# rongzhao-zhang/EfficientQ

Measured on AMD Instinct MI355X. Metric: ptq_calibration_throughput, higher is better.
Workload: dtype i8xi8->i32 (exact) for the Gram systems and per-iteration loss convs of the layers with quantised input, f32/f64 elsewhere

## Files before the change

efficientq_amd/_lib.py:

```python
from __future__ import annotations

import ctypes as C
import os

import torch

_HERE = os.path.dirname(os.path.abspath(__file__))
LIB_PATH = os.path.join(_HERE, "libeffq_hip.so")

EFFQ_OK = 0
_ERR_NAMES = {1: "EFFQ_ERR_ARG", 2: "EFFQ_ERR_HIP", 3: "EFFQ_ERR_WORKSPACE", 4: "EFFQ_ERR_NO_DEVICE",
              5: "EFFQ_ERR_NOT_CONVERGED"}


class EffqError(RuntimeError):
    pass


class Geom(C.Structure):
    _fields_ = [(n, C.c_int32) for n in
                ("N", "C1", "C2", "D", "H", "W", "KD", "KH", "KW", "SD", "SH", "SW", "PD", "PH", "PW")]

    def out_dims(self):
        return ((self.D + 2 * self.PD - self.KD) // self.SD + 1,
# ... 72 lines not shown
    "effq_fp_bracket_update": (_I, [_SZ, _I, _D, _D, _D, _I, _P, _P, _P]),
    "effq_fp_traj_max": (_SZ, []),
    "effq_fp_traj_ws_bytes": (_SZ, [_SZ]),
    "effq_spd_inverse_prepare": (_I, [_P]),
    "effq_fp_traj_pred_bytes": (_SZ, []),
    "effq_fixed_point_traj": (_I, [_P, _P, _P, _SZ, _I, _D, _D, _D, _I, _P, _P, _P, _SZ, _P]),
    "effq_fixed_point_bucket_rec": (_I, [_P, _P, _P, _SZ, _I, _D, _D, _D, _I, _P, _P, _SZ, _P, _P]),
    "effq_fixed_point_coop_rec": (_I, [_P, _P, _P, _SZ, _I, _D, _D, _D, _I, _P, _P, _P, _P]),
    "effq_fp_check": (_I, [_P, _P, _P]),
    "effq_fp_channels_max_row": (_I, []),
    "effq_fixed_point_channels": (_I, [_P, _P, _P, _I, _I, _I, _D, _I, _P, _P, _P, _P]),
    "effq_fixed_point_channels_proj": (_I, [_P, _P, _P, _I, _I, _I, _D, _I, _P, _P, _P, _P, _F, _P, _P, _P, _I, _I, _D,
                                            _D, _P]),
    "effq_gram_packed_elems": (_SZ, [_I, _I]),
    "effq_gram_pack": (_I, [_P, _P, _I, _I, _P, _P]),
    "effq_gram_unpack": (_I, [_P, _I, _I, _P, _P, _P]),
    "effq_act_quant_backward": (_I, [_P, _P, _I, _P, _P, _P, _SZ, _P, _P]),
    "effq_att_classes_ws_bytes": (_SZ, []),
    "effq_att_classes": (_I, [_P, _LL, _P, _P, _P, C.POINTER(C.c_int32), _P, _P]),
    "effq_prof_enable": (_I, [_I]),
    "effq_prof_count": (_I, []),
    "effq_prof_read": (_I, [_I, C.POINTER(ProfRecord)]),
    "effq_admm_num_inverses": (_I, [_D, _D, _I, _I]),
    "effq_admm_run": (_I, [C.POINTER(AdmmRunArgs)]),
    "effq_admm_select_best": (_I, [_P, _I, _P, _P, _SZ, _SZ, _P, _P, _P, _P]),
    "effq_gram_ws_bytes": (_SZ, [_GP, _I]),
    "effq_gram_accum": (_I, [_P, _P, _P, _GP, _I, _P, _P, _I, _P, _SZ, _P]),
    "effq_gram_plan_query": (_I, [_GP, _I, _IP, _IP, _IP, _IP, _LLP, _IP, _IP]),
    "effq_gram_i8_supported": (_I, [_GP, _I]),
    "effq_gram_i8_ws_bytes": (_SZ, [_GP, _I]),
    "effq_gram_accum_i8": (_I, [_P, _P, _GP, _I, _P, _I, _P, _P, _P, _I, _LL, _P, _P, _I, _P, _SZ, _P]),
    "effq_gram_accum_i8_unw": (_I, [_P, _P, _GP, _I, _P, _I, _P, _P, _P, _I, _LL, _P, _P, _I, _P, _P, _P, _SZ, _P]),
    "effq_gram_i8_plan_query": (_I, [_GP, _I, _LL, _IP, _IP, _IP, _IP, _IP, _IP]),
    "effq_upsample_trilinear": (_I, [_P, _I, _I, _I, _I, _I, _I, _I, _I, _P, _P]),
    "effq_gram_f64_supported": (_I, [_GP, _I]),
    "effq_gram_f64_ws_bytes": (_SZ, [_GP, _I]),
    "effq_gram_f64": (_I, [_P, _P, _GP, _I, _P, _P, _P, _SZ, _P]),
    "effq_gram_f64_plan_query": (_I, [_GP, _I, _IP, _IP, _IP, _IP]),
    "effq_gram_loss_ws_bytes": (_SZ, [_I]),
    "effq_gram_loss": (_I, [_P, _P, _P, _P, _P, _I, _I, _I, _P, _P, _SZ, _P]),
    "effq_packed_bytes": (_SZ, [_SZ, _I]),
    "effq_pack_levels": (_I, [_P, _SZ, _I, _P, _P]),
    "effq_unpack_levels": (_I, [_P, _SZ, _I, _P, _P]),
    "effq_ainv_ld": (_I, [_I]),
    "effq_fp_bracket_export_words": (_SZ, []),
    "effq_fp_bracket_export": (_I, [_P, _SZ, _P, _P, _SZ, _P]),
    "effq_fp_bracket_rebase": (_I, [_P, _P, _SZ, _P]),
    "effq_fp_bracket_import": (_I, [_P, _SZ, _P, _I, _SZ, _P, _P, _SZ, _P]),
    "effq_admm_uses_traj": (_I, [_SZ, _I]),
    "effq_gram_loss_i8_supported": (_I, [_I, _I, _I, _I]),
    "effq_gram_loss_i8_num_planes": (_I, [C.c_longlong]),
    "effq_gram_loss_i8_planes_bytes": (_SZ, [_I, _I, _I]),
    "effq_gram_loss_i8_prepare": (_I, [_P, _I, _I, _P, _I, _I, _P, _P, _P]),
    "effq_gram_loss_i8_ws_bytes": (_SZ, []),
    "effq_gram_loss_i8": (_I, [_P, _I, _P, _P, _P, _P, _P, _P, _P, _I, _I, _I, _I, _I, _I, _P, _P, _SZ, _P]),
    "effq_spd_inverse_ws_bytes": (_SZ, [_I]),
    "effq_spd_inverse": (_I, [_P, _I, _I, _D, _D, _P, _P, _SZ, _P]),
    "effq_spd_inverse_plan": (_I, [_I, _IP, _IP, _IP]),
    "effq_prox_plan_query": (_I, [_I, _I, _IP, _IP, _IP, _IP]),
    "effq_prox_ws_bytes": (_SZ, [_I, _I]),
    "effq_prox_solve": (_I, [_P, _P, _P, _P, _P, _P, _I, _I, _I, _D, _D, _P, _P, _P, _SZ, _P]),
    "effq_prox_solve_shifted": (_I, [_P, _P, _P, _P, _P, _P, _I, _I, _I, _D, _D, _D, _I, _P, _P, _P, _SZ, _P]),
    "effq_admm_presum": (_I, [_P, _P, _P, _SZ, _P]),
    "effq_admm_project_dual": (_I, [_P, _P, _P, _I, _P, _P, _F, _P, _SZ, _P]),
    "effq_conv_i8_supported": (_I, [_GP, _I, _I]),
    "effq_conv_i8s_supported": (_I, [_GP, _I, _I]),
# ... 84 lines not shown
```

efficientq_amd/csrc/gram_i8.hip:

```cpp
#include <stdint.h>
#include <stdlib.h>
#include "common.h"

namespace effq {

typedef int gi_v4i __attribute__((ext_vector_type(4)));
typedef int gi_v16i __attribute__((ext_vector_type(16)));

constexpr int GI_KC = 128;
constexpr int GI_MB = 128;
constexpr int GI_RS = GI_KC + 16;
constexpr int GI_T = 256;
constexpr int GI_PANEL = GI_MB * GI_RS;
constexpr int GI_LDS = 4 * GI_PANEL + 2 * GI_KC * 16;
constexpr int GI_MAXCLS = 16;
constexpr int GI_MAX_CPS = 1000;

struct GramI8Params {
  const uint8_t* x;
  const int8_t* yd;
  const int* vox_list;
  const int* chunk_cls;
  const int* vtab;
  int N, C1, C2, C2P, D, H, W, OD, OH, OW;
  int KD, KH, KW, SD, SH, SW, PD, PH, PW;
  int T, RX, YR0, E, NB, NBX, npairs;
  long long V;
  int nchunks, nsplit, cps, ncls;
  long long* slabs;
  int debug;
};

__device__ __forceinline__ void gi_transpose4(int r0, int r1, int r2, int r3, int (&o)[4]) {
  const int t0 = __builtin_amdgcn_perm(r1, r0, 0x05010400);
  const int t1 = __builtin_amdgcn_perm(r1, r0, 0x07030602);
  const int t2 = __builtin_amdgcn_perm(r3, r2, 0x05010400);
  const int t3 = __builtin_amdgcn_perm(r3, r2, 0x07030602);
  o[0] = __builtin_amdgcn_perm(t2, t0, 0x05040100);
  o[1] = __builtin_amdgcn_perm(t2, t0, 0x07060302);
  o[2] = __builtin_amdgcn_perm(t3, t1, 0x05040100);
  o[3] = __builtin_amdgcn_perm(t3, t1, 0x07060302);
}

__device__ __forceinline__ gi_v4i gi_build_entry(const GramI8Params& p, int v) {
  gi_v4i e = {0, 0, 0, 0};
  if (v < 0) return e;
  int t = v;
  const int ow = t % p.OW;
  t /= p.OW;
  const int oh = t % p.OH;
  t /= p.OH;
  const int od = t % p.OD;
  const int n = t / p.OD;
  const int id0 = od * p.SD - p.PD, ih0 = oh * p.SH - p.PH, iw0 = ow * p.SW - p.PW;
  unsigned m = 0x80000000u;
  int tap = 0;
  for (int kd = 0; kd < p.KD; ++kd)
    for (int kh = 0; kh < p.KH; ++kh)
      for (int kw = 0; kw < p.KW; ++kw, ++tap) {
        const int id = id0 + kd, ih = ih0 + kh, iw = iw0 + kw;
        const bool ok = id >= 0 && id < p.D && ih >= 0 && ih < p.H && iw >= 0 && iw < p.W;
        m |= (ok ? 1u : 0u) << tap;
      }
  e[0] = ((n * p.D + id0) * p.H + ih0) * p.W + iw0;
  e[1] = (int)m;
  e[2] = v;
  return e;
}

__global__ __launch_bounds__(256) void k_gi_voxtable(GramI8Params p, gi_v4i* __restrict__ table) {
  const long long nslots = (long long)p.nchunks * GI_KC;
  const long long stride = (long long)gridDim.x * blockDim.x;
  for (long long s = (long long)blockIdx.x * blockDim.x + threadIdx.x; s < nslots; s += stride) {
    const int v = (p.vox_list != nullptr) ? p.vox_list[s] : ((s < p.V) ? (int)s : -1);
    table[s] = gi_build_entry(p, v);
  }
}

__global__ __launch_bounds__(GI_T, 2) void k_gram_i8(GramI8Params p) {
  extern __shared__ __attribute__((aligned(16))) unsigned char gi_smem[];
  unsigned char* const panI = gi_smem;
  unsigned char* const panJ = gi_smem + 2 * GI_PANEL;
  gi_v4i* const tbl = reinterpret_cast<gi_v4i*>(gi_smem + 4 * GI_PANEL);

  const int tid = threadIdx.x, lane = tid & 63, wid = tid >> 6;
  const int li = lane & 31, lh = lane >> 5;
  const int wr = wid >> 1, wc = wid & 1;

  int I = 0, rem = blockIdx.x;
  while (rem >= p.NB - I) {
    rem -= p.NB - I;
    ++I;
  }
  const int J = I + rem;
  const bool diag = (I == J);

  const int c_begin = blockIdx.y * p.cps;
  const int c_end = min(c_begin + p.cps, p.nchunks);
  if (c_begin >= c_end) return;

  const int vg = tid & 31, rg = tid >> 5;
  int kindI, tapI, offI, kindJ, tapJ, offJ;
  auto make_rg = [&](int r0, int& kind, int& tap, int& off) {
    kind = 3;
    tap = 0;
    off = 0;
    if (r0 < p.RX) {
      kind = 0;
      tap = r0 / p.C1;
      const int c0 = r0 - tap * p.C1;
      const int kw = tap % p.KW, t2 = tap / p.KW;
      const int kh = t2 % p.KH, kd = t2 / p.KH;
      off = ((kd * p.H + kh) * p.W + kw) * p.C1 + c0;
    } else if (r0 == p.RX) {
      kind = 2;
    } else if (r0 >= p.YR0 && r0 < p.E) {
      kind = 1;
      off = r0 - p.YR0;
    }
  };
  make_rg(I * GI_MB + 16 * rg, kindI, tapI, offI);
  make_rg(J * GI_MB + 16 * rg, kindJ, tapJ, offJ);
  const unsigned char* const srcI = (kindI == 1) ? reinterpret_cast<const unsigned char*>(p.yd) : p.x;
  const unsigned char* const srcJ = (kindJ == 1) ? reinterpret_cast<const unsigned char*>(p.yd) : p.x;
  const int ystride = 4 * p.C2P;

  const gi_v4i* const vtab = reinterpret_cast<const gi_v4i*>(p.vtab);

  gi_v4i vI[4], vJ[4];
  unsigned okI = 0, okJ = 0;
#define GI_FETCH(val, okb, kind, tap, off, src, slot)                                            \
  {                                                                                              \
    okb = 0;                                                                                     \
    _Pragma("unroll") for (int q = 0; q < 4; ++q) {                                              \
      const gi_v4i e = tbl[(slot) * GI_KC + vg + 32 * q];                                        \
      const unsigned m = (unsigned)e[1];                                                         \
      const unsigned okx = (m >> (tap)) & 1u, okv = m >> 31;                                     \
      const unsigned ok = (kind == 0) ? okx : ((kind <= 2) ? okv : 0u);                          \
      const int ax = okx ? (e[0] * p.C1 + (off)) : 0;                                            \
      const int ay = e[2] * ystride + (off);                                                     \
      const int addr = (kind == 0) ? ax : ((kind == 1) ? ay : 0);                                \
      val[q] = *reinterpret_cast<const gi_v4i*>(src + ((EFFQ_DBG(p) == 2) ? 0 : addr));             \
      okb |= ok << q;                                                                            \
    }                                                                                            \
  }
  auto stage = [&](unsigned char* P, gi_v4i (&val)[4], unsigned okb, int kind) {
#pragma unroll
    for (int q = 0; q < 4; ++q) {
      const bool ok = (okb >> q) & 1u;
      gi_v4i z = {0, 0, 0, 0};
      if (kind == 2) z[0] = 1;
      if (!ok || kind >= 2) val[q] = ok ? z : gi_v4i{0, 0, 0, 0};
    }
#pragma unroll
    for (int k = 0; k < 4; ++k) {
      int o[4];
      gi_transpose4(val[0][k], val[1][k], val[2][k], val[3][k], o);
#pragma unroll
      for (int b = 0; b < 4; ++b) *reinterpret_cast<int*>(P + (16 * rg + 4 * k + b) * GI_RS + 4 * vg) = o[b];
    }
  };

  gi_v16i acc[2][2];
#pragma unroll
  for (int m = 0; m < 2; ++m)
#pragma unroll
    for (int n = 0; n < 2; ++n)
#pragma unroll
      for (int r = 0; r < 16; ++r) acc[m][n][r] = 0;
  const bool live = (I * GI_MB + wr * 64 < p.E) && (J * GI_MB + wc * 64 < p.E);

  auto flush = [&](int cls) {
    long long* S = p.slabs + ((size_t)cls * p.npairs + blockIdx.x) * (size_t)(GI_MB * GI_MB);
#pragma unroll
    for (int m = 0; m < 2; ++m)
#pragma unroll
      for (int n = 0; n < 2; ++n)
#pragma unroll
        for (int r = 0; r < 16; ++r) {
          const int row = wr * 64 + m * 32 + (r & 3) + 8 * (r >> 2) + 4 * lh;
          const int col = wc * 64 + n * 32 + li;
          const int v = acc[m][n][r];
          if (v != 0)
            atomicAdd(reinterpret_cast<unsigned long long*>(&S[row * GI_MB + col]), (unsigned long long)(long long)v);
          acc[m][n][r] = 0;
        }
  };

  {
    const int k = tid & (GI_KC - 1);
    const int cc = (tid < GI_KC) ? c_begin : min(c_begin + 1, c_end - 1);
    tbl[(tid < GI_KC ? 0 : 1) * GI_KC + k] = vtab[(size_t)cc * GI_KC + k];
  }
  __syncthreads();
// ... 11 lines not shown
    const int b = (c - c_begin) & 1;
    const int c2 = min(c + 2, c_end - 1);
    const int cls_raw = clsp[has_cls ? c2 : 0];
    const gi_v4i traw = vtab[(size_t)c2 * GI_KC + (tid & (GI_KC - 1))];
    GI_FETCH(vI, okI, kindI, tapI, offI, srcI, b ^ 1)
    if (!diag) GI_FETCH(vJ, okJ, kindJ, tapJ, offJ, srcJ, b ^ 1)
    __builtin_amdgcn_sched_barrier(0);
    if (live && EFFQ_DBG(p) != 1) {
      const unsigned char* PI = panI + b * GI_PANEL + (wr * 64 + li) * GI_RS + lh * 16;
      const unsigned char* PJ = (diag ? panI : panJ) + b * GI_PANEL + (wc * 64 + li) * GI_RS + lh * 16;
#pragma unroll
      for (int s = 0; s < GI_KC / 32; ++s) {
        gi_v4i a[2], bb[2];
#pragma unroll
        for (int m = 0; m < 2; ++m) a[m] = *reinterpret_cast<const gi_v4i*>(PI + m * 32 * GI_RS + s * 32);
#pragma unroll
        for (int n = 0; n < 2; ++n) bb[n] = *reinterpret_cast<const gi_v4i*>(PJ + n * 32 * GI_RS + s * 32);
#pragma unroll
        for (int m = 0; m < 2; ++m)
#pragma unroll
          for (int n = 0; n < 2; ++n) acc[m][n] = __builtin_amdgcn_mfma_i32_32x32x32_i8(a[m], bb[n], acc[m][n], 0, 0, 0);
      }
    }
    if (cls_next != cls_cur && live) flush(cls_cur);
    if (tid < GI_KC) tbl[b * GI_KC + tid] = traw;
    if (EFFQ_DBG(p) != 3) {
      stage(panI + (b ^ 1) * GI_PANEL, vI, okI, kindI);
      if (!diag) stage(panJ + (b ^ 1) * GI_PANEL, vJ, okJ, kindJ);
    }
    cls_cur = cls_next;
    cls_next = (c + 2 < c_end) ? (has_cls ? cls_raw : 0) : -1;
    __syncthreads();
  }
#undef GI_FETCH
}

__global__ __launch_bounds__(256) void k_gi_absmax(const float* __restrict__ y, size_t n, unsigned* __restrict__ out) {
  float m = 0.0f;
  const size_t stride = (size_t)gridDim.x * blockDim.x;
  for (size_t e = (size_t)blockIdx.x * blockDim.x + threadIdx.x; e < n; e += stride) m = fmaxf(m, fabsf(y[e]));
#pragma unroll
  for (int o = 32; o > 0; o >>= 1) m = fmaxf(m, __shfl_xor(m, o));
  if ((threadIdx.x & 63) == 0) atomicMax(out, __float_as_uint(m));
}

__device__ __forceinline__ int gi_y_exponent(unsigned ymax_bits) {
  const float ymax = __uint_as_float(ymax_bits);
  int ex = 0;
  if (ymax > 0.0f && ymax < 3.0e38f) (void)frexpf(ymax, &ex);
  return ex < -90 ? -90 : ex;
}

__global__ __launch_bounds__(256) void k_gi_ydigits(const float* __restrict__ y, long long V, int C2, int C2P,
                                                    const unsigned* __restrict__ ymax_bits, int8_t* __restrict__ yd) {
  const int ex = gi_y_exponent(*ymax_bits);
  const float scale = ldexpf(1.0f, 30 - ex);
  const size_t tot = (size_t)V * C2P, stride = (size_t)gridDim.x * blockDim.x;
  for (size_t e = (size_t)blockIdx.x * blockDim.x + threadIdx.x; e < tot; e += stride) {
    const size_t v = e / C2P;
    const int c = (int)(e - v * C2P);
    int d[4] = {0, 0, 0, 0};
    if (c < C2) {
      float f = y[v * C2 + c] * scale;
      if (!(fabsf(f) < 1.1e9f)) f = 0.0f;
      int t = (int)rintf(f);
#pragma unroll
      for (int k = 0; k < 3; ++k) {
// ... 87 lines not shown
  EFFQ_CHECK_ARG(ncls >= 1 && ncls <= GI_MAXCLS);
  GramI8Params& p = *pp;
  memset(&p, 0, sizeof(p));
  p.N = g->N; p.C1 = g->C1; p.C2 = g->C2; p.D = g->D; p.H = g->H; p.W = g->W;
  p.KD = g->KD; p.KH = g->KH; p.KW = g->KW; p.SD = g->SD; p.SH = g->SH; p.SW = g->SW;
  p.PD = g->PD; p.PH = g->PH; p.PW = g->PW;
  p.OD = (g->D + 2 * g->PD - g->KD) / g->SD + 1;
  p.OH = (g->H + 2 * g->PH - g->KH) / g->SH + 1;
  p.OW = (g->W + 2 * g->PW - g->KW) / g->SW + 1;
  EFFQ_CHECK_ARG(p.OD > 0 && p.OH > 0 && p.OW > 0);
  p.C2P = (g->C2 + 15) / 16 * 16;
  p.T = p.KD * p.KH * p.KW;
  p.RX = p.T * p.C1;
  p.YR0 = p.RX + 16;
  p.E = p.YR0 + 4 * p.C2P;
  p.NB = (p.E + GI_MB - 1) / GI_MB;
  p.NBX = (p.YR0 + GI_MB - 1) / GI_MB;
  p.npairs = p.NBX * p.NB - p.NBX * (p.NBX - 1) / 2;
  p.V = (long long)p.N * p.OD * p.OH * p.OW;
  EFFQ_CHECK_ARG((long long)g->N * g->D * g->H * g->W * g->C1 < (1ll << 31));
  EFFQ_CHECK_ARG(p.V * 4 * p.C2P < (1ll << 31));
  const long long nchunks = (n_list > 0) ? n_list / GI_KC : (p.V + GI_KC - 1) / GI_KC;
  EFFQ_CHECK_ARG(nchunks > 0 && nchunks < (1ll << 24));
  p.nchunks = (int)nchunks;
  p.ncls = ncls;
  long long want = (3072 + p.npairs - 1) / p.npairs;
  if (want > nchunks / 4) want = nchunks / 4;
  if (want < 1) want = 1;
  long long cps = (nchunks + want - 1) / want;
  if (cps > GI_MAX_CPS) cps = GI_MAX_CPS;
  p.cps = (int)cps;
  p.nsplit = (int)((nchunks + cps - 1) / cps);
  EFFQ_CHECK_ARG(p.nsplit <= 65535);
  return EFFQ_OK;
}

static size_t gram_i8_table_bytes(long long V, int ncls) { return (size_t)(V + (long long)GI_KC * (ncls + 1)) * 16; }

static size_t gram_i8_slab_bytes(const GramI8Params& p) {
  return (size_t)p.ncls * p.npairs * (size_t)(GI_MB * GI_MB) * sizeof(long long);
}

}

using namespace effq;

extern "C" {

int effq_gram_i8_supported(const effq_geom* g, int act_levels) {
  if (g == nullptr) return 0;
  if ((g->C1 % 16) != 0 || g->KD * g->KH * g->KW > 31 || g->KD < 1 || g->KH < 1 || g->KW < 1) return 0;
  if (act_levels < 2 || act_levels > 128) return 0;
  GramI8Params p;
  if (gram_i8_plan(g, 1, 0, &p) != EFFQ_OK) return 0;
  return 1;
}

size_t effq_gram_i8_ws_bytes(const effq_geom* g, int ncls) {
  GramI8Params p;
  if (gram_i8_plan(g, ncls, 0, &p) != EFFQ_OK) return 0;
  return 256 + gram_i8_slab_bytes(p) + (size_t)p.V * 4 * p.C2P + 256 + gram_i8_table_bytes(p.V, ncls) + 256;
}

int effq_gram_accum_i8_unw(const uint8_t* xidx_ndhwc, const float* y_ndhwc, const effq_geom* g, int has_bias,
                           const float* act_alpha_dev, int act_levels, const int32_t* vox_list, const int32_t* chunk_cls,
                           const float* cls_w_dev, int ncls, long long n_list, float* A0, float* B0, int accumulate,
// ... 15 lines not shown
  if (ws_bytes < need) {
    set_error("gram_i8: workspace %zu < required %zu", ws_bytes, need);
    return EFFQ_ERR_WORKSPACE;
  }
  char* base = reinterpret_cast<char*>(ws);
  unsigned* ymax = reinterpret_cast<unsigned*>(base);
  p.slabs = reinterpret_cast<long long*>(base + 256);
  int8_t* yd = reinterpret_cast<int8_t*>(base + 256 + slab_bytes);
  gi_v4i* vtab = reinterpret_cast<gi_v4i*>((reinterpret_cast<uintptr_t>(base + 256 + slab_bytes + (size_t)p.V * 4 * p.C2P) + 255) & ~(uintptr_t)255);
  p.x = xidx_ndhwc;
  p.yd = yd;
  p.vox_list = vox_list;
  p.chunk_cls = chunk_cls;
  p.vtab = reinterpret_cast<const int*>(vtab);
  p.debug = effq_ablate_env("EFFQ_GI8_DEBUG");
  hipStream_t st = as_stream(stream);
  EFFQ_HIP(hipMemsetAsync(base, 0, 256 + slab_bytes, st));
  const size_t ny = (size_t)p.V * p.C2;
  {
    size_t nb = (ny + 255) / 256;
    if (nb > 2048) nb = 2048;
    hipLaunchKernelGGL(k_gi_absmax, dim3((unsigned)nb), dim3(256), 0, st, y_ndhwc, ny, ymax);
    size_t nd = ((size_t)p.V * p.C2P + 255) / 256;
    if (nd > 8192) nd = 8192;
    hipLaunchKernelGGL(k_gi_ydigits, dim3((unsigned)nd), dim3(256), 0, st, y_ndhwc, p.V, p.C2, p.C2P, ymax, yd);
    EFFQ_LAUNCH_CHECK();
  }
  {
    size_t nt = ((size_t)p.nchunks * GI_KC + 255) / 256;
    if (nt > 4096) nt = 4096;
    hipLaunchKernelGGL(k_gi_voxtable, dim3((unsigned)nt), dim3(256), 0, st, p, vtab);
    EFFQ_LAUNCH_CHECK();
  }
  EFFQ_HIP(raise_lds_limit<k_gram_i8>(GI_LDS));
  hipLaunchKernelGGL(k_gram_i8, dim3((unsigned)p.npairs, (unsigned)p.nsplit), dim3(GI_T), GI_LDS, st, p);
  EFFQ_LAUNCH_CHECK();
  const int n = p.RX + (has_bias ? 1 : 0);
  size_t tot = (size_t)n * n + (size_t)p.C2 * n;
  size_t nb = (tot + 255) / 256;
  if (nb > 8192) nb = 8192;
  hipLaunchKernelGGL(k_gram_i8_finish, dim3((unsigned)nb), dim3(256), 0, st, p, n, has_bias ? 1 : 0, act_alpha_dev,
                     act_levels, ymax, cls_w_dev, A0, B0, accumulate, Au, Bu);
  EFFQ_LAUNCH_CHECK();
  return EFFQ_OK;
}

int effq_gram_i8_plan_query(const effq_geom* g, int ncls, long long n_list, int* nb, int* nbx, int* npairs, int* nchunks,
                            int* cps, int* nsplit) {
  EFFQ_CHECK_ARG(nb && nbx && npairs && nchunks && cps && nsplit && n_list >= 0 && (n_list % GI_KC) == 0);
  GramI8Params p;
  const int rc = gram_i8_plan(g, ncls, n_list, &p);
  if (rc != EFFQ_OK) return rc;
  *nb = p.NB;
  *nbx = p.NBX;
  *npairs = p.npairs;
  *nchunks = p.nchunks;
  *cps = p.cps;
  *nsplit = p.nsplit;
  return EFFQ_OK;
}

int effq_gram_accum_i8(const uint8_t* xidx_ndhwc, const float* y_ndhwc, const effq_geom* g, int has_bias,
                       const float* act_alpha_dev, int act_levels, const int32_t* vox_list, const int32_t* chunk_cls,
                       const float* cls_w_dev, int ncls, long long n_list, float* A0, float* B0, int accumulate,
                       void* ws, size_t ws_bytes, void* stream) {
  return effq_gram_accum_i8_unw(xidx_ndhwc, y_ndhwc, g, has_bias, act_alpha_dev, act_levels, vox_list, chunk_cls,
                                cls_w_dev, ncls, n_list, A0, B0, accumulate, nullptr, nullptr, ws, ws_bytes, stream);
}

}

namespace effq {
constexpr int CLS_SLOTS = 32;
constexpr int CLS_MAX = 16;
struct ClsTable {
  unsigned key[CLS_SLOTS];
  unsigned cnt[CLS_SLOTS];
  unsigned cursor[CLS_MAX];
  int overflow;
  int ncls;
  int n_list;
  int slot_cls[CLS_SLOTS];
  unsigned seg_start[CLS_MAX];
  float cls_w[CLS_MAX];
};

__device__ __forceinline__ int cls_find_or_insert(unsigned* keys, unsigned k) {
  unsigned h = (k * 2654435761u) >> 27;
  for (int probe = 0; probe < CLS_SLOTS; ++probe) {
    const unsigned cur = atomicCAS(&keys[h], 0xffffffffu, k);
// ... 2 lines not shown
  }
  return -1;
}

__global__ __launch_bounds__(256) void k_cls_count(const float* __restrict__ att, long long V, ClsTable* t) {
  __shared__ unsigned lkey[CLS_SLOTS], lcnt[CLS_SLOTS];
  __shared__ int lover;
  if (threadIdx.x < CLS_SLOTS) {
    lkey[threadIdx.x] = 0xffffffffu;
    lcnt[threadIdx.x] = 0u;
  }
  if (threadIdx.x == 0) lover = 0;
  __syncthreads();
  const long long stride = (long long)gridDim.x * blockDim.x;
  for (long long i = (long long)blockIdx.x * blockDim.x + threadIdx.x; i < V; i += stride) {
    const unsigned k = __float_as_uint(att[i]);
    const int sidx = (k == 0xffffffffu) ? -1 : cls_find_or_insert(lkey, k);
    if (sidx < 0)
      lover = 1;
    else
      atomicAdd(&lcnt[sidx], 1u);
  }
  __syncthreads();
  if (threadIdx.x < CLS_SLOTS && lkey[threadIdx.x] != 0xffffffffu) {
    const int g = cls_find_or_insert(t->key, lkey[threadIdx.x]);
    if (g < 0)
      t->overflow = 1;
    else
      atomicAdd(&t->cnt[g], lcnt[threadIdx.x]);
  }
  if (threadIdx.x == 0 && lover) t->overflow = 1;
}

__global__ void k_cls_layout(ClsTable* t, int* __restrict__ chunk_cls, int max_chunks) {
  int used[CLS_SLOTS], nu = 0;
  for (int sidx = 0; sidx < CLS_SLOTS; ++sidx)
    if (t->key[sidx] != 0xffffffffu) used[nu++] = sidx;
  if (nu > CLS_MAX) t->overflow = 1;
  if (t->overflow) {
    t->ncls = 0;
    t->n_list = 0;
    return;
  }
  for (int i = 1; i < nu; ++i) {
    const int sidx = used[i];
    const float v = __uint_as_float(t->key[sidx]);
    int j = i - 1;
    while (j >= 0 && __uint_as_float(t->key[used[j]]) > v) {
      used[j + 1] = used[j];
      --j;
    }
    used[j + 1] = sidx;
  }
  unsigned start = 0;
  int chunk = 0;
  for (int c = 0; c < nu; ++c) {
    const int sidx = used[c];
    t->slot_cls[sidx] = c;
    t->cls_w[c] = __uint_as_float(t->key[sidx]);
    t->seg_start[c] = start;
    t->cursor[c] = start;
    const unsigned padded = (t->cnt[sidx] + 127u) / 128u * 128u;
    for (unsigned q = 0; q < padded / 128u && chunk < max_chunks; ++q) chunk_cls[chunk++] = c;
    start += padded;
  }
  t->ncls = nu;
  t->n_list = (int)start;
}

__global__ __launch_bounds__(256) void k_cls_scatter(const float* __restrict__ att, long long V, ClsTable* t,
                                                     int* __restrict__ vox_list) {
  __shared__ unsigned lcnt[CLS_MAX], lbase[CLS_MAX];
  if (t->overflow) return;
  if (threadIdx.x < CLS_MAX) lcnt[threadIdx.x] = 0u;
  __syncthreads();
  const long long per = (V + gridDim.x - 1) / gridDim.x;
  const long long i0 = (long long)blockIdx.x * per, i1 = (i0 + per < V) ? i0 + per : V;
  for (long long i = i0 + threadIdx.x; i < i1; i += blockDim.x) {
    const unsigned k = __float_as_uint(att[i]);
    unsigned h = (k * 2654435761u) >> 27;
    while (t->key[h] != k) h = (h + 1) & (CLS_SLOTS - 1);
    atomicAdd(&lcnt[t->slot_cls[h]], 1u);
  }
  __syncthreads();
  if (threadIdx.x < CLS_MAX) {
    lbase[threadIdx.x] = (lcnt[threadIdx.x] != 0u) ? atomicAdd(&t->cursor[threadIdx.x], lcnt[threadIdx.x]) : 0u;
    lcnt[threadIdx.x] = 0u;
  }
  __syncthreads();
  for (long long i = i0 + threadIdx.x; i < i1; i += blockDim.x) {
    const unsigned k = __float_as_uint(att[i]);
    unsigned h = (k * 2654435761u) >> 27;
    while (t->key[h] != k) h = (h + 1) & (CLS_SLOTS - 1);
    const int c = t->slot_cls[h];
    vox_list[lbase[c] + atomicAdd(&lcnt[c], 1u)] = (int)i;
  }
}
}

extern "C" {

size_t effq_att_classes_ws_bytes(void) { return sizeof(ClsTable) + 64; }

int effq_att_classes(const float* att, long long V, int32_t* vox_list, int32_t* chunk_cls, float* cls_w_dev,
                     int32_t* info_host_out, void* ws, void* stream) {
  EFFQ_CHECK_ARG(att && vox_list && chunk_cls && cls_w_dev && info_host_out && ws && V > 0 && V < (1ll << 31) - 4096);
  hipStream_t st = as_stream(stream);
  ClsTable* t = reinterpret_cast<ClsTable*>(ws);
  EFFQ_HIP(hipMemsetAsync(t, 0, sizeof(ClsTable), st));
  EFFQ_HIP(hipMemsetAsync(t->key, 0xff, sizeof(t->key), st));
  const long long cap = V + 128 * CLS_MAX;
  EFFQ_HIP(hipMemsetAsync(vox_list, 0xff, sizeof(int32_t) * (size_t)cap, st));
  int blocks = (int)((V + 256 * 16 - 1) / (256 * 16));
  if (blocks > 2048) blocks = 2048;
  if (blocks < 1) blocks = 1;
  hipLaunchKernelGGL(k_cls_count, dim3(blocks), dim3(256), 0, st, att, V, t);
  hipLaunchKernelGGL(k_cls_layout, dim3(1), dim3(1), 0, st, t, chunk_cls, (int)(V / 128 + CLS_MAX));
  hipLaunchKernelGGL(k_cls_scatter, dim3(blocks), dim3(256), 0, st, att, V, t, vox_list);
  EFFQ_LAUNCH_CHECK();
  ClsTable host;
  EFFQ_HIP(hipMemcpyAsync(&host, t, sizeof(ClsTable), hipMemcpyDeviceToHost, st));
  EFFQ_HIP(hipStreamSynchronize(st));
  info_host_out[0] = host.ncls;
  info_host_out[1] = host.n_list;
  info_host_out[2] = host.overflow;
  if (!host.overflow) EFFQ_HIP(hipMemcpyAsync(cls_w_dev, t->cls_w, sizeof(float) * CLS_MAX, hipMemcpyDeviceToDevice, st));
  return EFFQ_OK;
}

}
```

efficientq_amd/hip_ops.py:

```python
from __future__ import annotations

import ctypes as C
import math
from typing import Optional, Tuple

import torch

from . import _lib
from ._lib import Geom, check

ADMM_TOL = 1e-5
FP_BRACKET_MIN = 1 << 18
DP_GATHER_AFTER = 4
DP_GATHER_MAX_BYTES = 128 << 20


def _ptr(t: Optional[torch.Tensor]):
    return None if t is None else C.c_void_p(t.data_ptr())


def to_ndhwc(x: torch.Tensor) -> torch.Tensor:
    return x.permute(0, 2, 3, 4, 1).contiguous()


# ... 344 lines not shown
    def gram(self, x_ndhwc: torch.Tensor, att: Optional[torch.Tensor], y_ndhwc: torch.Tensor, geom: Geom,
             has_bias: bool, A0: Optional[torch.Tensor] = None, B0: Optional[torch.Tensor] = None):
        x = self._f32(x_ndhwc)
        y = self._f32(y_ndhwc)
        a = self._f32(att) if att is not None else None
        _check_shapes(geom, x, y=y, att=a)
        n = geom.C1 * geom.KD * geom.KH * geom.KW + int(has_bias)
        acc = int(A0 is not None)
        if A0 is not None and (tuple(A0.shape) != (n, n) or tuple(B0.shape) != (geom.C2, n)):
            raise _lib.EffqError("gram: A0/B0 shapes do not match the geometry")
        if A0 is None:
            A0 = torch.empty(n, n, dtype=torch.float32, device=self.device)
            B0 = torch.empty(geom.C2, n, dtype=torch.float32, device=self.device)
        need = self.lib.effq_gram_ws_bytes(C.byref(geom), int(has_bias))
        ws = self._workspace("gram", need)
        check(self.lib.effq_gram_accum(_ptr(x), _ptr(a), _ptr(y), C.byref(geom), int(has_bias), _ptr(A0), _ptr(B0),
                                       acc, _ptr(ws), ws.numel(), self.stream), "effq_gram_accum")
        return A0, B0

    def gram_plan(self, geom: Geom, has_bias: bool) -> dict:
        vec, nb, npairs, nsplit, fold, fin = (C.c_int() for _ in range(6))
        vps = C.c_longlong()
        check(self.lib.effq_gram_plan_query(C.byref(geom), int(has_bias), C.byref(vec), C.byref(nb), C.byref(npairs),
                                            C.byref(nsplit), C.byref(vps), C.byref(fold), C.byref(fin)),
              "effq_gram_plan_query")
        return dict(vec=bool(vec.value), NB=nb.value, npairs=npairs.value, nsplit=nsplit.value, vox_per_split=vps.value,
                    fold=fold.value, finish_blocks=fin.value)

    def gram_i8_plan(self, geom: Geom, ncls: int = 1, n_list: int = 0) -> dict:
        out = [C.c_int() for _ in range(6)]
        check(self.lib.effq_gram_i8_plan_query(C.byref(geom), int(ncls), int(n_list), *[C.byref(o) for o in out]),
              "effq_gram_i8_plan_query")
        return dict(zip(("NB", "NBX", "npairs", "nchunks", "cps", "nsplit"), (o.value for o in out)))

    def gram_f64_plan(self, geom: Geom, has_bias: bool) -> dict:
        out = [C.c_int() for _ in range(4)]
        check(self.lib.effq_gram_f64_plan_query(C.byref(geom), int(has_bias), *[C.byref(o) for o in out]),
              "effq_gram_f64_plan_query")
        return dict(zip(("nchunk", "grid", "ntiles", "tpw"), (o.value for o in out)))

    def gram_i8_supported(self, geom: Geom, act_levels: int) -> bool:
        return bool(self.lib.effq_gram_i8_supported(C.byref(geom), int(act_levels)))

    GRAM_I8_MAX_CLASSES = 16

    def att_classes(self, att: Optional[torch.Tensor]):
        if att is None:
            return (None, None, None, 1)
        key = (att.data_ptr(), att.numel(), att._version)
        hit = self._att_cache.get(key)
        if hit is not None:
            return hit[1]
        flat = self._f32(att).reshape(-1)
        V = flat.numel()
        lst = torch.empty(V + 128 * self.GRAM_I8_MAX_CLASSES, dtype=torch.int32, device=flat.device)
        chunk_cls = torch.empty(V // 128 + self.GRAM_I8_MAX_CLASSES, dtype=torch.int32, device=flat.device)
        cls_w = torch.empty(self.GRAM_I8_MAX_CLASSES, dtype=torch.float32, device=flat.device)
        info = (C.c_int32 * 3)()
        ws = self._workspace("att_cls", self.lib.effq_att_classes_ws_bytes())
        check(self.lib.effq_att_classes(_ptr(flat), V, _ptr(lst), _ptr(chunk_cls), _ptr(cls_w), info, _ptr(ws),
                                        self.stream), "effq_att_classes")
        k, n_list, overflow = int(info[0]), int(info[1]), int(info[2])
        res = None if overflow else (lst[:n_list], chunk_cls[: n_list // 128], cls_w[:k], k)
        if len(self._att_cache) > 16:
            self._att_cache.clear()
        self._att_cache[key] = (att, res)
# ... 1037 lines not shown
```

include/effq_hip.h:

```cpp
#ifndef EFFQ_HIP_H
#define EFFQ_HIP_H

#include <stddef.h>
#include <stdint.h>

#ifdef __cplusplus
extern "C" {
#endif

enum {
  EFFQ_OK = 0,
  EFFQ_ERR_ARG = 1,
  EFFQ_ERR_HIP = 2,
  EFFQ_ERR_WORKSPACE = 3,
  EFFQ_ERR_NO_DEVICE = 4,
  EFFQ_ERR_NOT_CONVERGED = 5
};

typedef struct effq_geom {
  int32_t N, C1, C2;
  int32_t D, H, W;
  int32_t KD, KH, KW;
  int32_t SD, SH, SW;
  int32_t PD, PH, PW;
// ... 70 lines not shown
int effq_fp_bracket_export(const void* ws, size_t n, long long* out, float* list_out, size_t list_cap, void* stream);
int effq_fp_bracket_import(const void* ws_src, size_t n_src, const long long* pack_dev, int world, size_t list_cap,
                           effq_fp_state* state_dev, void* ws_dst, size_t ws_dst_bytes, void* stream);
int effq_fp_bracket_rebase(effq_fp_state* state_dev, void* ws, size_t n, void* stream);
int effq_fp_channels_max_row(void);
int effq_fixed_point_channels(const float* a, const float* b, float* v_out, int c2, int nwrow, int levels, double tol,
                              int max_iter, double* alpha_out, int32_t* iters_out, int32_t* err_flag_dev, void* stream);
int effq_fixed_point_channels_proj(const float* wstar, float* dual, float* v_out, int c2, int nwrow, int levels,
                                   double tol, int max_iter, double* alpha_out, int32_t* iters_out, int32_t* err_flag_dev,
                                   float* G, float dual_div, float* Bm, const float* B0, const float* W0, int n, int ldb,
                                   double rho_next, double eta, void* stream);

int effq_fp_check(const effq_fp_state* state_dev, int32_t* err_flag_dev, void* stream);

size_t effq_gram_ws_bytes(const effq_geom* g, int has_bias);
int effq_gram_accum(const float* x_ndhwc, const float* att, const float* y_ndhwc, const effq_geom* g,
                    int has_bias, float* A0, float* B0, int accumulate, void* ws, size_t ws_bytes,
                    void* stream);
int effq_gram_plan_query(const effq_geom* g, int has_bias, int* vec, int* nb, int* npairs, int* nsplit,
                         long long* vox_per_split, int* fold, int* finish_blocks);

int effq_gram_i8_supported(const effq_geom* g, int act_levels);
size_t effq_gram_i8_ws_bytes(const effq_geom* g, int ncls);
int effq_gram_accum_i8(const uint8_t* xidx_ndhwc, const float* y_ndhwc, const effq_geom* g, int has_bias,
                       const float* act_alpha_dev, int act_levels, const int32_t* vox_list,
                       const int32_t* chunk_cls, const float* cls_w_dev, int ncls, long long n_list,
                       float* A0, float* B0, int accumulate, void* ws, size_t ws_bytes, void* stream);
int effq_gram_accum_i8_unw(const uint8_t* xidx_ndhwc, const float* y_ndhwc, const effq_geom* g, int has_bias,
                           const float* act_alpha_dev, int act_levels, const int32_t* vox_list, const int32_t* chunk_cls,
                           const float* cls_w_dev, int ncls, long long n_list, float* A0, float* B0, int accumulate,
                           double* Au, double* Bu, void* ws, size_t ws_bytes, void* stream);
int effq_gram_i8_plan_query(const effq_geom* g, int ncls, long long n_list, int* nb, int* nbx, int* npairs, int* nchunks,
                            int* cps, int* nsplit);

int effq_gram_f64_supported(const effq_geom* g, int has_bias);
size_t effq_gram_f64_ws_bytes(const effq_geom* g, int has_bias);
int effq_gram_f64(const float* x_ndhwc, const float* y_ndhwc, const effq_geom* g, int has_bias, double* Au, double* Bu,
                  void* ws, size_t ws_bytes, void* stream);
int effq_gram_f64_plan_query(const effq_geom* g, int has_bias, int* nchunk, int* grid, int* ntiles, int* tpw);

size_t effq_gram_loss_ws_bytes(int n);
int effq_gram_loss(const double* Au, const double* Bu, const double* syy_dev, const float* G, const float* b, int c2, int n,
                   int has_bias, double* sqerr_out, void* ws, size_t ws_bytes, void* stream);

int effq_gram_loss_i8_supported(int c2, int n, int has_bias, int w_levels);
int effq_gram_loss_i8_num_planes(long long kmax);
size_t effq_gram_loss_i8_planes_bytes(int n, int has_bias, int nplanes);
int effq_gram_loss_i8_prepare(const double* Au, int n, int has_bias, const float* act_alpha_dev, int act_levels,
                              int nplanes, int8_t* planes, int32_t* err_flag_dev, void* stream);
size_t effq_gram_loss_i8_ws_bytes(void);
int effq_gram_loss_i8(const int8_t* planes, int nplanes, const double* Au, const double* Bu, const double* syy_dev,
                      const int8_t* Gq, const float* b, const effq_fp_state* states, const float* act_alpha_dev,
                      int act_levels, int w_levels, int c2, int n, int has_bias, int count, double* hist_out, void* ws,
                      size_t ws_bytes, void* stream);


size_t effq_att_classes_ws_bytes(void);
int effq_att_classes(const float* att, long long V, int32_t* vox_list, int32_t* chunk_cls, float* cls_w_dev,
                     int32_t* info_host_out, void* ws, void* stream);

int effq_spd_inverse_prepare(void* stream);
int effq_ainv_ld(int n);
size_t effq_spd_inverse_ws_bytes(int n);
int effq_spd_inverse(const float* A0, int n, int has_bias, double rho, double eta, float* Ainv,
                     void* ws, size_t ws_bytes, void* stream);
int effq_spd_inverse_plan(int n, int* wide, int* nblk, int* pivot_blocks);
// ... 192 lines not shown
```

Measured before the change: 25.07.

## Add wide 256x256 super-tile int8 Gram kernel and parallelise class layout

Adds a 512-thread Gram kernel that computes a 2x2 group of 128x128 block pairs per workgroup. Each staged panel is reused across more MFMA tiles, and a split-phase schedule lets half the waves stage the next chunk while the other half compute. It is selected when the block count lies in a middle range. Separately, the single-thread class-layout kernel now fills chunk_cls with many threads, with one thread per block still doing the sort. The cost is larger LDS use and lower occupancy, plus wasted work on edge and diagonal super-tiles.

Result: no change. 25.05 (-0.1%).

```diff
diff --git a/efficientq_amd/_lib.py b/efficientq_amd/_lib.py
--- a/efficientq_amd/_lib.py
+++ b/efficientq_amd/_lib.py
@@ -128,6 +128,7 @@
     "effq_gram_accum_i8": (_I, [_P, _P, _GP, _I, _P, _I, _P, _P, _P, _I, _LL, _P, _P, _I, _P, _SZ, _P]),
     "effq_gram_accum_i8_unw": (_I, [_P, _P, _GP, _I, _P, _I, _P, _P, _P, _I, _LL, _P, _P, _I, _P, _P, _P, _SZ, _P]),
     "effq_gram_i8_plan_query": (_I, [_GP, _I, _LL, _IP, _IP, _IP, _IP, _IP, _IP]),
+    "effq_gram_i8_tile_query": (_I, [_GP, _I, _LL, _IP, _IP, _IP]),
     "effq_upsample_trilinear": (_I, [_P, _I, _I, _I, _I, _I, _I, _I, _I, _P, _P]),
     "effq_gram_f64_supported": (_I, [_GP, _I]),
     "effq_gram_f64_ws_bytes": (_SZ, [_GP, _I]),
diff --git a/efficientq_amd/csrc/gram_i8.hip b/efficientq_amd/csrc/gram_i8.hip
--- a/efficientq_amd/csrc/gram_i8.hip
+++ b/efficientq_amd/csrc/gram_i8.hip
@@ -14,6 +14,12 @@
 constexpr int GI_PANEL = GI_MB * GI_RS;
 constexpr int GI_LDS = 4 * GI_PANEL + 2 * GI_KC * 16;
 constexpr int GI_MAXCLS = 16;
+constexpr int GW_MB = 2 * GI_MB;
+constexpr int GW_T = 512;
+constexpr int GW_PANEL = GW_MB * GI_RS;
+constexpr int GW_LDS = 4 * GW_PANEL + 4 * GI_KC * 16;
+constexpr int GW_MIN_NB = 4;
+constexpr int GW_MAX_NB = 48;
 constexpr int GI_MAX_CPS = 1000;
 
 struct GramI8Params {
@@ -25,6 +31,7 @@
   int N, C1, C2, C2P, D, H, W, OD, OH, OW;
   int KD, KH, KW, SD, SH, SW, PD, PH, PW;
   int T, RX, YR0, E, NB, NBX, npairs;
+  int wide, NS, NSX, nsuper;
   long long V;
   int nchunks, nsplit, cps, ncls;
   long long* slabs;
@@ -77,58 +84,25 @@
   }
 }
 
-__global__ __launch_bounds__(GI_T, 2) void k_gram_i8(GramI8Params p) {
-  extern __shared__ __attribute__((aligned(16))) unsigned char gi_smem[];
-  unsigned char* const panI = gi_smem;
-  unsigned char* const panJ = gi_smem + 2 * GI_PANEL;
-  gi_v4i* const tbl = reinterpret_cast<gi_v4i*>(gi_smem + 4 * GI_PANEL);
-
-  const int tid = threadIdx.x, lane = tid & 63, wid = tid >> 6;
-  const int li = lane & 31, lh = lane >> 5;
-  const int wr = wid >> 1, wc = wid & 1;
-
-  int I = 0, rem = blockIdx.x;
-  while (rem >= p.NB - I) {
-    rem -= p.NB - I;
-    ++I;
-  }
-  const int J = I + rem;
-  const bool diag = (I == J);
-
-  const int c_begin = blockIdx.y * p.cps;
-  const int c_end = min(c_begin + p.cps, p.nchunks);
-  if (c_begin >= c_end) return;
-
-  const int vg = tid & 31, rg = tid >> 5;
-  int kindI, tapI, offI, kindJ, tapJ, offJ;
-  auto make_rg = [&](int r0, int& kind, int& tap, int& off) {
-    kind = 3;
-    tap = 0;
-    off = 0;
-    if (r0 < p.RX) {
-      kind = 0;
-      tap = r0 / p.C1;
-      const int c0 = r0 - tap * p.C1;
-      const int kw = tap % p.KW, t2 = tap / p.KW;
-      const int kh = t2 % p.KH, kd = t2 / p.KH;
-      off = ((kd * p.H + kh) * p.W + kw) * p.C1 + c0;
-    } else if (r0 == p.RX) {
-      kind = 2;
-    } else if (r0 >= p.YR0 && r0 < p.E) {
-      kind = 1;
-      off = r0 - p.YR0;
-    }
-  };
-  make_rg(I * GI_MB + 16 * rg, kindI, tapI, offI);
-  make_rg(J * GI_MB + 16 * rg, kindJ, tapJ, offJ);
-  const unsigned char* const srcI = (kindI == 1) ? reinterpret_cast<const unsigned char*>(p.yd) : p.x;
-  const unsigned char* const srcJ = (kindJ == 1) ? reinterpret_cast<const unsigned char*>(p.yd) : p.x;
-  const int ystride = 4 * p.C2P;
-
-  const gi_v4i* const vtab = reinterpret_cast<const gi_v4i*>(p.vtab);
-
-  gi_v4i vI[4], vJ[4];
-  unsigned okI = 0, okJ = 0;
+__device__ __forceinline__ void gi_row_group(const GramI8Params& p, int r0, int& kind, int& tap, int& off) {
+  kind = 3;
+  tap = 0;
+  off = 0;
+  if (r0 < p.RX) {
+    kind = 0;
+    tap = r0 / p.C1;
+    const int c0 = r0 - tap * p.C1;
+    const int kw = tap % p.KW, t2 = tap / p.KW;
+    const int kh = t2 % p.KH, kd = t2 / p.KH;
+    off = ((kd * p.H + kh) * p.W + kw) * p.C1 + c0;
+  } else if (r0 == p.RX) {
+    kind = 2;
+  } else if (r0 >= p.YR0 && r0 < p.E) {
+    kind = 1;
+    off = r0 - p.YR0;
+  }
+}
+
 #define GI_FETCH(val, okb, kind, tap, off, src, slot)                                            \
   {                                                                                              \
     okb = 0;                                                                                     \
@@ -144,22 +118,59 @@
       okb |= ok << q;                                                                            \
     }                                                                                            \
   }
-  auto stage = [&](unsigned char* P, gi_v4i (&val)[4], unsigned okb, int kind) {
-#pragma unroll
-    for (int q = 0; q < 4; ++q) {
-      const bool ok = (okb >> q) & 1u;
-      gi_v4i z = {0, 0, 0, 0};
-      if (kind == 2) z[0] = 1;
-      if (!ok || kind >= 2) val[q] = ok ? z : gi_v4i{0, 0, 0, 0};
-    }
-#pragma unroll
-    for (int k = 0; k < 4; ++k) {
-      int o[4];
-      gi_transpose4(val[0][k], val[1][k], val[2][k], val[3][k], o);
-#pragma unroll
-      for (int b = 0; b < 4; ++b) *reinterpret_cast<int*>(P + (16 * rg + 4 * k + b) * GI_RS + 4 * vg) = o[b];
-    }
-  };
+
+__device__ __forceinline__ void gi_stage(unsigned char* P, gi_v4i (&val)[4], unsigned okb, int kind, int rg, int vg) {
+#pragma unroll
+  for (int q = 0; q < 4; ++q) {
+    const bool ok = (okb >> q) & 1u;
+    gi_v4i z = {0, 0, 0, 0};
+    if (kind == 2) z[0] = 1;
+    if (!ok || kind >= 2) val[q] = ok ? z : gi_v4i{0, 0, 0, 0};
+  }
+#pragma unroll
+  for (int k = 0; k < 4; ++k) {
+    int o[4];
+    gi_transpose4(val[0][k], val[1][k], val[2][k], val[3][k], o);
+#pragma unroll
+    for (int b = 0; b < 4; ++b) *reinterpret_cast<int*>(P + (16 * rg + 4 * k + b) * GI_RS + 4 * vg) = o[b];
+  }
+}
+
+__global__ __launch_bounds__(GI_T, 2) void k_gram_i8(GramI8Params p) {
+  extern __shared__ __attribute__((aligned(16))) unsigned char gi_smem[];
+  unsigned char* const panI = gi_smem;
+  unsigned char* const panJ = gi_smem + 2 * GI_PANEL;
+  gi_v4i* const tbl = reinterpret_cast<gi_v4i*>(gi_smem + 4 * GI_PANEL);
+
+  const int tid = threadIdx.x, lane = tid & 63, wid = tid >> 6;
+  const int li = lane & 31, lh = lane >> 5;
+  const int wr = wid >> 1, wc = wid & 1;
+
+  int I = 0, rem = blockIdx.x;
+  while (rem >= p.NB - I) {
+    rem -= p.NB - I;
+    ++I;
+  }
+  const int J = I + rem;
+  const bool diag = (I == J);
+
+  const int c_begin = blockIdx.y * p.cps;
+  const int c_end = min(c_begin + p.cps, p.nchunks);
+  if (c_begin >= c_end) return;
+
+  const int vg = tid & 31, rg = tid >> 5;
+  int kindI, tapI, offI, kindJ, tapJ, offJ;
+  gi_row_group(p, I * GI_MB + 16 * rg, kindI, tapI, offI);
+  gi_row_group(p, J * GI_MB + 16 * rg, kindJ, tapJ, offJ);
+  const unsigned char* const srcI = (kindI == 1) ? reinterpret_cast<const unsigned char*>(p.yd) : p.x;
+  const unsigned char* const srcJ = (kindJ == 1) ? reinterpret_cast<const unsigned char*>(p.yd) : p.x;
+  const int ystride = 4 * p.C2P;
+
+  const gi_v4i* const vtab = reinterpret_cast<const gi_v4i*>(p.vtab);
+
+  gi_v4i vI[4], vJ[4];
+  unsigned okI = 0, okJ = 0;
+  auto stage = [&](unsigned char* P, gi_v4i (&val)[4], unsigned okb, int kind) { gi_stage(P, val, okb, kind, rg, vg); };
 
   gi_v16i acc[2][2];
 #pragma unroll
@@ -237,7 +248,135 @@
     cls_next = (c + 2 < c_end) ? (has_cls ? cls_raw : 0) : -1;
     __syncthreads();
   }
-#undef GI_FETCH
+}
+
+__global__ __launch_bounds__(GW_T) void k_gram_i8_w(GramI8Params p) {
+  extern __shared__ __attribute__((aligned(16))) unsigned char gi_smem[];
+  unsigned char* const panI = gi_smem;
+  unsigned char* const panJ = gi_smem + 2 * GW_PANEL;
+  gi_v4i* const tbl = reinterpret_cast<gi_v4i*>(gi_smem + 4 * GW_PANEL);
+
+  const int tid = threadIdx.x, lane = tid & 63, wid = tid >> 6;
+  const int li = lane & 31, lh = lane >> 5;
+  const int wr = wid >> 1, wc = wid & 1;
+
+  int SI = 0, rem = blockIdx.x;
+  while (rem >= p.NS - SI) {
+    rem -= p.NS - SI;
+    ++SI;
+  }
+  const int SJ = SI + rem;
+  const bool diag = (SI == SJ);
+
+  const int c_begin = blockIdx.y * p.cps;
+  const int c_end = min(c_begin + p.cps, p.nchunks);
+  if (c_begin >= c_end) return;
+
+  const int I = 2 * SI + (wr >> 1), J = 2 * SJ + wc;
+  const bool live = I < p.NBX && J < p.NB && I <= J && (I * GI_MB + (wr & 1) * 64 < p.E);
+  const int pidx = I * p.NB - I * (I - 1) / 2 + (J - I);
+
+  const int vg = tid & 31, rg = tid >> 5;
+  int kindI, tapI, offI, kindJ, tapJ, offJ;
+  gi_row_group(p, SI * GW_MB + 16 * rg, kindI, tapI, offI);
+  gi_row_group(p, SJ * GW_MB + 16 * rg, kindJ, tapJ, offJ);
+  if (!diag && 2 * SI + (rg >> 3) >= p.NBX) kindI = 3;
+  const unsigned char* const srcI = (kindI == 1) ? reinterpret_cast<const unsigned char*>(p.yd) : p.x;
+  const unsigned char* const srcJ = (kindJ == 1) ? reinterpret_cast<const unsigned char*>(p.yd) : p.x;
+  const int ystride = 4 * p.C2P;
+
+  const gi_v4i* const vtab = reinterpret_cast<const gi_v4i*>(p.vtab);
+
+  gi_v4i vI[4], vJ[4];
+  unsigned okI = 0, okJ = 0;
+
+  gi_v16i acc[2][4];
+#pragma unroll
+  for (int m = 0; m < 2; ++m)
+#pragma unroll
+    for (int n = 0; n < 4; ++n)
+#pragma unroll
+      for (int r = 0; r < 16; ++r) acc[m][n][r] = 0;
+
+  auto flush = [&](int cls) {
+    long long* S = p.slabs + ((size_t)cls * p.npairs + pidx) * (size_t)(GI_MB * GI_MB);
+#pragma unroll
+    for (int m = 0; m < 2; ++m)
+#pragma unroll
+      for (int n = 0; n < 4; ++n)
+#pragma unroll
+        for (int r = 0; r < 16; ++r) {
+          const int row = (wr & 1) * 64 + m * 32 + (r & 3) + 8 * (r >> 2) + 4 * lh;
+          const int col = n * 32 + li;
+          const int v = acc[m][n][r];
+          if (v != 0)
+            atomicAdd(reinterpret_cast<unsigned long long*>(&S[row * GI_MB + col]), (unsigned long long)(long long)v);
+          acc[m][n][r] = 0;
+        }
+  };
+
+  const int half = wid >> 2;
+  const int nloc = c_end - c_begin;
+  if (tid < 3 * GI_KC) {
+    const int k = tid & (GI_KC - 1), j = tid >> 7;
+    tbl[j * GI_KC + k] = vtab[(size_t)min(c_begin + j, c_end - 1) * GI_KC + k];
+  }
+  __syncthreads();
+  GI_FETCH(vI, okI, kindI, tapI, offI, srcI, 0)
+  if (!diag) GI_FETCH(vJ, okJ, kindJ, tapJ, offJ, srcJ, 0)
+  gi_stage(panI, vI, okI, kindI, rg, vg);
+  if (!diag) gi_stage(panJ, vJ, okJ, kindJ, rg, vg);
+  if (nloc > 1) {
+    GI_FETCH(vI, okI, kindI, tapI, offI, srcI, 1)
+    if (!diag) GI_FETCH(vJ, okJ, kindJ, tapJ, offJ, srcJ, 1)
+  }
+  __syncthreads();
+
+  const bool has_cls = p.chunk_cls != nullptr;
+  const int* const clsp = has_cls ? p.chunk_cls : reinterpret_cast<const int*>(p.x);
+  int cls_cur = has_cls ? clsp[c_begin] : 0;
+  int cls_next = (nloc > 1) ? (has_cls ? clsp[c_begin + 1] : 0) : -1;
+
+  for (int t = 0; t < 2 * nloc; ++t) {
+    const int i = t >> 1, ph = t & 1;
+    if (half == ph) {
+      const int b = i & 1;
+      gi_v4i traw = {0, 0, 0, 0};
+      if (tid < GI_KC) traw = vtab[(size_t)min(c_begin + i + 3, c_end - 1) * GI_KC + tid];
+      if (live && EFFQ_DBG(p) != 1) {
+        const unsigned char* PI = panI + b * GW_PANEL + (wr * 64 + li) * GI_RS + lh * 16;
+        const unsigned char* PJ = (diag ? panI : panJ) + b * GW_PANEL + (wc * 128 + li) * GI_RS + lh * 16;
+#pragma unroll
+        for (int s = 0; s < GI_KC / 32; ++s) {
+          gi_v4i a[2], bb[4];
+#pragma unroll
+          for (int m = 0; m < 2; ++m) a[m] = *reinterpret_cast<const gi_v4i*>(PI + m * 32 * GI_RS + s * 32);
+#pragma unroll
+          for (int n = 0; n < 4; ++n) bb[n] = *reinterpret_cast<const gi_v4i*>(PJ + n * 32 * GI_RS + s * 32);
+#pragma unroll
+          for (int m = 0; m < 2; ++m)
+#pragma unroll
+            for (int n = 0; n < 4; ++n) acc[m][n] = __builtin_amdgcn_mfma_i32_32x32x32_i8(a[m], bb[n], acc[m][n], 0, 0, 0);
+        }
+      }
+      if (cls_next != cls_cur && live) flush(cls_cur);
+      if (tid < GI_KC) tbl[((i + 3) & 3) * GI_KC + tid] = traw;
+      cls_cur = cls_next;
+      const int c2 = c_begin + i + 2;
+      cls_next = (c2 < c_end) ? (has_cls ? clsp[c2] : 0) : -1;
+    } else {
+      if (i + 1 < nloc && EFFQ_DBG(p) != 3) {
+        gi_stage(panI + ((i + 1) & 1) * GW_PANEL, vI, okI, kindI, rg, vg);
+        if (!diag) gi_stage(panJ + ((i + 1) & 1) * GW_PANEL, vJ, okJ, kindJ, rg, vg);
+      }
+      if (i + 2 < nloc) {
+        const int slot = (i + 2) & 3;
+        GI_FETCH(vI, okI, kindI, tapI, offI, srcI, slot)
+        if (!diag) GI_FETCH(vJ, okJ, kindJ, tapJ, offJ, srcJ, slot)
+      }
+    }
+    __syncthreads();
+  }
 }
 
 __global__ __launch_bounds__(256) void k_gi_absmax(const float* __restrict__ y, size_t n, unsigned* __restrict__ out) {
@@ -391,6 +530,10 @@
   p.cps = (int)cps;
   p.nsplit = (int)((nchunks + cps - 1) / cps);
   EFFQ_CHECK_ARG(p.nsplit <= 65535);
+  p.wide = p.NB >= GW_MIN_NB && p.NB < GW_MAX_NB;
+  p.NS = (p.NB + 1) / 2;
+  p.NSX = (p.NBX + 1) / 2;
+  p.nsuper = p.NSX * p.NS - p.NSX * (p.NSX - 1) / 2;
   return EFFQ_OK;
 }
 
@@ -472,8 +615,13 @@
     hipLaunchKernelGGL(k_gi_voxtable, dim3((unsigned)nt), dim3(256), 0, st, p, vtab);
     EFFQ_LAUNCH_CHECK();
   }
-  EFFQ_HIP(raise_lds_limit<k_gram_i8>(GI_LDS));
-  hipLaunchKernelGGL(k_gram_i8, dim3((unsigned)p.npairs, (unsigned)p.nsplit), dim3(GI_T), GI_LDS, st, p);
+  if (p.wide) {
+    EFFQ_HIP(raise_lds_limit<k_gram_i8_w>(GW_LDS));
+    hipLaunchKernelGGL(k_gram_i8_w, dim3((unsigned)p.nsuper, (unsigned)p.nsplit), dim3(GW_T), GW_LDS, st, p);
+  } else {
+    EFFQ_HIP(raise_lds_limit<k_gram_i8>(GI_LDS));
+    hipLaunchKernelGGL(k_gram_i8, dim3((unsigned)p.npairs, (unsigned)p.nsplit), dim3(GI_T), GI_LDS, st, p);
+  }
   EFFQ_LAUNCH_CHECK();
   const int n = p.RX + (has_bias ? 1 : 0);
   size_t tot = (size_t)n * n + (size_t)p.C2 * n;
@@ -496,6 +644,17 @@
   *npairs = p.npairs;
   *nchunks = p.nchunks;
   *cps = p.cps;
+  *nsplit = p.nsplit;
+  return EFFQ_OK;
+}
+
+int effq_gram_i8_tile_query(const effq_geom* g, int ncls, long long n_list, int* wide, int* ntiles, int* nsplit) {
+  EFFQ_CHECK_ARG(wide && ntiles && nsplit && n_list >= 0 && (n_list % GI_KC) == 0);
+  GramI8Params p;
+  const int rc = gram_i8_plan(g, ncls, n_list, &p);
+  if (rc != EFFQ_OK) return rc;
+  *wide = p.wide;
+  *ntiles = p.wide ? p.nsuper : p.npairs;
   *nsplit = p.nsplit;
   return EFFQ_OK;
 }
@@ -564,40 +723,62 @@
   if (threadIdx.x == 0 && lover) t->overflow = 1;
 }
 
-__global__ void k_cls_layout(ClsTable* t, int* __restrict__ chunk_cls, int max_chunks) {
-  int used[CLS_SLOTS], nu = 0;
-  for (int sidx = 0; sidx < CLS_SLOTS; ++sidx)
-    if (t->key[sidx] != 0xffffffffu) used[nu++] = sidx;
-  if (nu > CLS_MAX) t->overflow = 1;
-  if (t->overflow) {
-    t->ncls = 0;
-    t->n_list = 0;
-    return;
-  }
-  for (int i = 1; i < nu; ++i) {
-    const int sidx = used[i];
-    const float v = __uint_as_float(t->key[sidx]);
-    int j = i - 1;
-    while (j >= 0 && __uint_as_float(t->key[used[j]]) > v) {
-      used[j + 1] = used[j];
-      --j;
+__global__ __launch_bounds__(256) void k_cls_layout(ClsTable* t, int* __restrict__ chunk_cls, int max_chunks) {
+  __shared__ unsigned first_chunk[CLS_MAX + 1];
+  __shared__ int nused;
+  if (threadIdx.x == 0) {
+    const bool wr = blockIdx.x == 0;
+    int used[CLS_SLOTS], nu = 0;
+    for (int sidx = 0; sidx < CLS_SLOTS; ++sidx)
+      if (t->key[sidx] != 0xffffffffu) used[nu++] = sidx;
+    if (nu > CLS_MAX || t->overflow) {
+      nu = 0;
+      if (wr) {
+        t->overflow = 1;
+        t->ncls = 0;
+        t->n_list = 0;
+      }
+    } else {
+      for (int i = 1; i < nu; ++i) {
+        const int sidx = used[i];
+        const float v = __uint_as_float(t->key[sidx]);
+        int j = i - 1;
+        while (j >= 0 && __uint_as_float(t->key[used[j]]) > v) {
+          used[j + 1] = used[j];
+          --j;
+        }
+        used[j + 1] = sidx;
+      }
+      unsigned start = 0;
+      for (int c = 0; c < nu; ++c) {
+        const int sidx = used[c];
+        first_chunk[c] = start / 128u;
+        if (wr) {
+          t->slot_cls[sidx] = c;
+          t->cls_w[c] = __uint_as_float(t->key[sidx]);
+          t->seg_start[c] = start;
+          t->cursor[c] = start;
+        }
+        start += (t->cnt[sidx] + 127u) / 128u * 128u;
+      }
+      first_chunk[nu] = start / 128u;
+      if (wr) {
+        t->ncls = nu;
+        t->n_list = (int)start;
+      }
     }
-    used[j + 1] = sidx;
-  }
-  unsigned start = 0;
-  int chunk = 0;
-  for (int c = 0; c < nu; ++c) {
-    const int sidx = used[c];
-    t->slot_cls[sidx] = c;
-    t->cls_w[c] = __uint_as_float(t->key[sidx]);
-    t->seg_start[c] = start;
-    t->cursor[c] = start;
-    const unsigned padded = (t->cnt[sidx] + 127u) / 128u * 128u;
-    for (unsigned q = 0; q < padded / 128u && chunk < max_chunks; ++q) chunk_cls[chunk++] = c;
-    start += padded;
-  }
-  t->ncls = nu;
-  t->n_list = (int)start;
+    nused = nu;
+  }
+  __syncthreads();
+  const int nu = nused;
+  if (nu == 0) return;
+  unsigned total = first_chunk[nu];
+  if (total > (unsigned)max_chunks) total = (unsigned)max_chunks;
+  for (unsigned q = blockIdx.x * blockDim.x + threadIdx.x; q < total; q += gridDim.x * blockDim.x) {
+    int c = 0;
+    while (first_chunk[c + 1] <= q) ++c;
+    chunk_cls[q] = c;
+  }
 }
 
 __global__ __launch_bounds__(256) void k_cls_scatter(const float* __restrict__ att, long long V, ClsTable* t,
@@ -647,7 +828,10 @@
   if (blocks > 2048) blocks = 2048;
   if (blocks < 1) blocks = 1;
   hipLaunchKernelGGL(k_cls_count, dim3(blocks), dim3(256), 0, st, att, V, t);
-  hipLaunchKernelGGL(k_cls_layout, dim3(1), dim3(1), 0, st, t, chunk_cls, (int)(V / 128 + CLS_MAX));
+  const int max_chunks = (int)(V / 128 + CLS_MAX);
+  int lblocks = (max_chunks + 1023) / 1024;
+  if (lblocks > 64) lblocks = 64;
+  hipLaunchKernelGGL(k_cls_layout, dim3(lblocks), dim3(256), 0, st, t, chunk_cls, max_chunks);
   hipLaunchKernelGGL(k_cls_scatter, dim3(blocks), dim3(256), 0, st, att, V, t, vox_list);
   EFFQ_LAUNCH_CHECK();
   ClsTable host;
diff --git a/efficientq_amd/hip_ops.py b/efficientq_amd/hip_ops.py
--- a/efficientq_amd/hip_ops.py
+++ b/efficientq_amd/hip_ops.py
@@ -400,6 +400,13 @@
         check(self.lib.effq_gram_i8_plan_query(C.byref(geom), int(ncls), int(n_list), *[C.byref(o) for o in out]),
               "effq_gram_i8_plan_query")
         return dict(zip(("NB", "NBX", "npairs", "nchunks", "cps", "nsplit"), (o.value for o in out)))
+
+    def gram_i8_tiles(self, geom: Geom, ncls: int = 1, n_list: int = 0) -> dict:
+        out = [C.c_int() for _ in range(3)]
+        check(self.lib.effq_gram_i8_tile_query(C.byref(geom), int(ncls), int(n_list), *[C.byref(o) for o in out]),
+              "effq_gram_i8_tile_query")
+        wide, ntiles, nsplit = (o.value for o in out)
+        return dict(kernel="k_gram_i8_w" if wide else "k_gram_i8", ntiles=ntiles, nsplit=nsplit)
 
     def gram_f64_plan(self, geom: Geom, has_bias: bool) -> dict:
         out = [C.c_int() for _ in range(4)]
diff --git a/include/effq_hip.h b/include/effq_hip.h
--- a/include/effq_hip.h
+++ b/include/effq_hip.h
@@ -126,6 +126,7 @@
                            double* Au, double* Bu, void* ws, size_t ws_bytes, void* stream);
 int effq_gram_i8_plan_query(const effq_geom* g, int ncls, long long n_list, int* nb, int* nbx, int* npairs, int* nchunks,
                             int* cps, int* nsplit);
+int effq_gram_i8_tile_query(const effq_geom* g, int ncls, long long n_list, int* wide, int* ntiles, int* nsplit);
 
 int effq_gram_f64_supported(const effq_geom* g, int has_bias);
 size_t effq_gram_f64_ws_bytes(const effq_geom* g, int has_bias);
```
